# calf-ai/calfkit-sdk

Measured on NVIDIA H100. Metric: agent_events_per_sec, higher is better.
Workload: dtype u8

## Files before the change

### calfkit-sdk_b200/csrc/ck_kernels.cuh

```cuda
#ifndef CK_KERNELS_CUH
#define CK_KERNELS_CUH

#include <cuda_runtime.h>
#include "ck_walk.cuh"
#include "ck_canon.cuh"

#if !defined(__CUDA_ARCH__)
extern __shared__ uint4 ck_win_smem[];
#endif

#ifndef CK_HIST_MIN
#define CK_HIST_MIN 2048u
#endif
#ifndef CK_LONG_MIN
#define CK_LONG_MIN 16384u
#endif
struct ck_canon_ctl { unsigned long long cursor; u32 count; u32 elems; u32 cand; u32 cand_next; };
struct ck_view {
    const u8* in; const long long* off;
    const u8* ovl; const long long* ovl_off; const u32* ovl_len;
    ck_canon_ctl* canon_ctl; u32* canon_list;
    const u32* perm;
    const uint2* hist_skip;
    ck_elem* elems; u32 elem_cap;
    const u32* len;
};
__device__ __forceinline__ const u8* ck_rec_in(const ck_view& v, u32 i, u32& len) {
    long long a = v.off[i];
    len = v.len ? v.len[i] : (u32)(v.off[i + 1] - a);
    return v.in + a;
}
__device__ __forceinline__ const u8* ck_rec(const ck_view& v, u32 i, u32& len) {
    long long o = v.ovl_off[i];
    if (o >= 0) { len = v.ovl_len[i]; return v.ovl + o; }
    return ck_rec_in(v, i, len);
}

#define CK_TPL_MAX_PARTS 6
struct ck_tool_cfg {
    int32_t  publish_topic_id;
    uint32_t tpl_nparts;
    uint32_t tpl_kind[CK_TPL_MAX_PARTS];
    uint32_t tpl_off[CK_TPL_MAX_PARTS];
    uint32_t tpl_len[CK_TPL_MAX_PARTS];
    uint32_t lit_comma_q[2];
    uint32_t lit_q[2];
    uint32_t lit_open[2];
    uint32_t lit_mid[2];
    uint32_t lit_close[2];
    uint32_t lit_value_open[2];
};

struct ck_pub {
    uint32_t payload;
    int32_t  topic_id;
    uint32_t topic_off, topic_len;
    uint32_t record;
    uint32_t has_key;
    int32_t  partition;
    uint32_t pad;
};

struct ck_topic_table {
    uint32_t cap;
    const uint32_t* hash;
    const int32_t*  id;
    const uint32_t* name_off;
    const uint32_t* name_len;
    const uint8_t*  names;
};

__device__ __forceinline__ u32 ck_fnv1a(const u8* p, u32 n) {
    u32 h = 2166136261u;
    for (u32 i = 0; i < n; i++) h = (h ^ p[i]) * 16777619u;
    return h ? h : 1u;
}

#define CK_WALK_THREADS 128
template <class R>
__device__ __forceinline__ void ck_walk_one(ck_view v, u32 n, u32* __restrict__ cols, u32 stride, u32 mode) {
    u32 i = blockIdx.x * blockDim.x + threadIdx.x;
    if (i >= n) return;
    if (v.perm) i = v.perm[i];
    u32 len; const u8* rec;
    if (mode == 0) rec = ck_rec_in(v, i, len);
    else { if (v.ovl_off[i] < 0) return; rec = ck_rec(v, i, len); }
    uint2 skip = make_uint2(0u, 0u);
    if (mode == 0 && len >= CK_HIST_MIN && v.hist_skip) skip = v.hist_skip[i];
    if (skip.x == 0xffffffffu) return;
    WalkOut o; o.base = cols + i; o.stride = stride; o.skip_open = skip.x; o.skip_close = skip.y;
    u32 status, stop = 0;
    if (len == 0) status = CK_EMPTY;
    else {
        R r; r.init(rec, len);
        AnyCtx cx;
        cx.kfill = 0;
        status = ck_walk_envelope(r, o, cx, stop) ? CK_OK : (mode ? CK_UNSUPPORTED : CK_NOT_CANONICAL);
    }
    o.set(CK_COL_STATUS, status);
    o.set(CK_COL_ERR, stop);
    if (mode == 0 && status == CK_NOT_CANONICAL && v.canon_ctl) {
        u32 k = atomicAdd(&v.canon_ctl->count, 1u);
        v.canon_list[k] = i;
    }
}
#ifndef CK_WALK_MINB
#define CK_WALK_MINB 8
#endif
__global__ void __launch_bounds__(256)
ck_classify_kernel(ck_view v, u32 n, u32* __restrict__ cand) {
    u32 j = blockIdx.x * blockDim.x + threadIdx.x;
    bool take = false; u32 i = 0;
    if (j < n) { i = v.perm ? v.perm[j] : j; u32 len; ck_rec_in(v, i, len); take = len >= CK_HIST_MIN; }
    u32 m = __ballot_sync(0xffffffffu, take);
    if (!m) return;
    u32 lane = threadIdx.x & 31, base = 0;
    if (lane == (u32)(__ffs(m) - 1)) base = atomicAdd(&v.canon_ctl->cand, (u32)__popc(m));
    base = __shfl_sync(0xffffffffu, base, __ffs(m) - 1);
    if (take) cand[base + __popc(m & ((1u << lane) - 1u))] = i;
}
__global__ void __launch_bounds__(CK_WALK_THREADS, CK_WALK_MINB)
ck_walk_kernel(ck_view v, u32 n, u32* __restrict__ cols, u32 stride, u32 mode) { ck_walk_one<WRd>(v, n, cols, stride, mode); }
__global__ void __launch_bounds__(CK_WALK_THREADS, 8)
ck_walk_global_kernel(ck_view v, u32 n, u32* __restrict__ cols, u32 stride, u32 mode) { ck_walk_one<GRd>(v, n, cols, stride, mode); }

__global__ void __launch_bounds__(64)
ck_canon_kernel(ck_view v, u32 n, u32* __restrict__ cols, u32 stride, u8* __restrict__ ovl, long long ovl_cap,
                long long* __restrict__ ovl_off, u32* __restrict__ ovl_len) {
    u32 cnt = v.canon_ctl->count;
    for (u32 k = blockIdx.x * blockDim.x + threadIdx.x; k < cnt; k += gridDim.x * blockDim.x) {
        u32 i = v.canon_list[k];
        u32 len, out_len = 0;
        const u8* src = ck_rec_in(v, i, len);
        u32 st = ck_canonicalise(src, len, nullptr, 0, out_len);
        if (st != CK_OK) { cols[(size_t)CK_COL_STATUS * stride + i] = st; continue; }
        u32 need = (out_len + 15u) & ~15u;
        long long o0 = (long long)atomicAdd(&v.canon_ctl->cursor, (unsigned long long)need);
        if (o0 + need > ovl_cap) { cols[(size_t)CK_COL_STATUS * stride + i] = CK_UNSUPPORTED; continue; }
        st = ck_canonicalise(src, len, ovl + o0, need, out_len);
        if (st != CK_OK) { cols[(size_t)CK_COL_STATUS * stride + i] = CK_UNSUPPORTED; continue; }
        for (u32 b = out_len; b < need; b++) ovl[o0 + b] = 0;
        ovl_len[i] = out_len;
        ovl_off[i] = o0;
    }
}

__global__ void __launch_bounds__(64)
ck_rewalk_list_kernel(ck_view v, u32 n, u32* __restrict__ cols, u32 stride) {
    u32 cnt = v.canon_ctl->count;
    for (u32 k = blockIdx.x * blockDim.x + threadIdx.x; k < cnt; k += gridDim.x * blockDim.x) {
        u32 i = v.canon_list[k];
        if (v.ovl_off[i] < 0) continue;
        u32 len; const u8* rec = ck_rec(v, i, len);
        WalkOut o; o.base = cols + i; o.stride = stride;
        u32 stop = 0;
        GRdT r; r.init(rec, len);
        AnyCtx cx; cx.kfill = 0;
        u32 status = ck_walk_envelope(r, o, cx, stop) ? CK_OK : CK_UNSUPPORTED;
        o.set(CK_COL_STATUS, status);
        o.set(CK_COL_ERR, stop);
    }
}

__device__ __forceinline__ bool ck_span_eq(Rd& r, u32 a, u32 b, u32 len) {
    for (u32 k = 0; k < len; k++) if (r.at(a + k) != r.at(b + k)) return false;
    return true;
}

__device__ __forceinline__ Span ck_dict_find(Rd& r, u32 obj, u32 key_off, u32 key_len) {
    u32 pos = obj + 1;
    Span none = {0, 0};
    while (pos < r.n && r.at(pos) != '}') {
        Span k;
        if (!ck_string(r, pos, k)) return none;
        pos++;
        u32 v = pos;
        ck_skip_value(r, pos);
        if (k.len == key_len && ck_span_eq(r, k.off, key_off, key_len)) { Span s = {v, pos - v}; return s; }
        if (pos < r.n && r.at(pos) == ',') pos++;
    }
    return none;
}

#ifndef CK_PLAN_PF
#define CK_PLAN_PF 1
#endif
#ifndef CK_PLAN_MINB
#define CK_PLAN_MINB 1
#endif
__device__ __forceinline__ void ck_prefetch_l2(const u8* p) {
#if CK_PLAN_PF == 2
    asm volatile("prefetch.global.L1 [%0];" :: "l"(p));
#else
    asm volatile("prefetch.global.L2 [%0];" :: "l"(p));
#endif
}
#define CK_DIRECT_MIN 48u
struct SegWriter {
    ck_out_desc* d;
    Rd* r; const u8* lit; const u8* aux; u8* slot;
    u32 n, total;
    bool in_glue, overflow;
    u32 gfill, grun;
    unsigned long long acc; u32 cnt;

    __device__ __forceinline__ void init(ck_out_desc* dd, Rd* rr, const u8* l, const u8* a, u8* s) {
        d = dd; r = rr; lit = l; aux = a; slot = s; n = 0; total = 0; in_glue = false; overflow = false; gfill = 0; grun = 0; acc = 0; cnt = 0;
    }
    __device__ __forceinline__ void seg(u32 src, u32 off, u32 len) {
        if (n < CK_MAX_SEGS) { d->seg[n][0] = off; d->seg[n][1] = (len << 2) | src; n++; } else overflow = true;
    }
    __device__ __forceinline__ void put8(unsigned long long chunk, u32 nb) {
        if (gfill + nb > CK_GLUE_STRIDE) { overflow = true; return; }
        if (nb < 8) chunk &= (~0ull >> (8 * (8 - nb)));
        acc |= chunk << (8 * cnt);
        u32 c2 = cnt + nb;
        gfill += nb;
        if (c2 >= 8) {
            *(unsigned long long*)(slot + ((gfill - (c2 - 8)) - 8)) = acc;
            acc = cnt ? (chunk >> (8 * (8 - cnt))) : 0ull;
            c2 -= 8;
        }
        cnt = c2;
    }
    __device__ __forceinline__ void put(u8 b) { put8((unsigned long long)b, 1); }
    __device__ __forceinline__ static unsigned long long load8_g(const u8* p) {
        u32 s = (u32)((uintptr_t)p & 7);
        const unsigned long long* q = (const unsigned long long*)((uintptr_t)p - s);
        unsigned long long lo = q[0];
        if (s == 0) return lo;
        unsigned long long hi = q[1];
        return (lo >> (8 * s)) | (hi << (64 - 8 * s));
    }
    __device__ __forceinline__ unsigned long long fetch8(u32 src, u32 off) {
        return src == CK_SRC_INPUT ? r->load8(off) : load8_g((src == CK_SRC_LIT ? lit : aux) + off);
    }
    __device__ __forceinline__ void close_run() {
        if (cnt) { *(unsigned long long*)(slot + (gfill & ~7u)) = acc; acc = 0; cnt = 0; }
        seg(CK_SRC_GLUE, grun, gfill - grun);
        gfill = (gfill + 15u) & ~15u;
        in_glue = false;
    }
    __device__ __forceinline__ void glue_bytes(u32 src, u32 off, u32 len) {
        if (!in_glue) { in_glue = true; grun = gfill; }
        for (u32 k = 0; k < len; k += 8) put8(fetch8(src, off + k), len - k < 8 ? len - k : 8);
        total += len;
    }
    __device__ __forceinline__ void add(u32 src, u32 off, u32 len) {
        if (len == 0) return;
        bool direct_ok = (src == CK_SRC_INPUT || src == CK_SRC_AUX) && len >= CK_DIRECT_MIN;
        if (!direct_ok) { glue_bytes(src, off, len); return; }
        if (in_glue || (total & 15u)) {
            u32 need = (16u - (total & 15u)) & 15u;
            glue_bytes(src, off, need);
            off += need; len -= need;
            close_run();
        }
        u32 body = len & ~15u;
        seg(src, off, body);
        total += body;
// ... 565 lines not shown
```

### calfkit-sdk_b200/csrc/ck_walk.cuh

```cuda
#ifndef CK_WALK_CUH
#define CK_WALK_CUH

#include "ck_common.h"

#if defined(__CUDACC__)
#define CK_HD __host__ __device__ __forceinline__
#define CK_HD_NOINLINE __host__ __device__ __noinline__
#else
#define CK_HD inline __attribute__((always_inline))
#define CK_HD_NOINLINE __attribute__((noinline))
#endif

typedef uint8_t u8;
typedef uint32_t u32;
typedef uint64_t u64;
#if !defined(__CUDACC__)
struct uint4 { u32 x, y, z, w; };
#endif

struct Span { u32 off, len; };

#if defined(__CUDA_ARCH__)
extern __shared__ uint4 ck_win_smem[];
#endif
#define CK_LX_SEP 640u
#define CK_LX_CLOSE 320u
#define CK_LX_MIN 4u
#define CK_LX_KEYS 128u
#define CK_DEFER_MAX 4096u
#define CK_LX_OPEN 8u
struct ck_elem { u32 rec, start, end; };
struct ck_long_index {
    u32 n_sep[2], n_close[2], ok, rec, defer_cap, n_open;
    u32 open_sq[CK_LX_OPEN];
    ck_elem* defer_list; u32* defer_ctr;
    u32 sep[2][CK_LX_SEP];
    u32 close_[2][CK_LX_CLOSE];
    u32 kh[2][CK_LX_KEYS], koff[2][CK_LX_KEYS];
};
#if defined(__CUDA_ARCH__)
CK_HD u32 ck_lane() { return threadIdx.x & 31u; }
CK_HD bool ck_all(bool p) { return __all_sync(0xffffffffu, p); }
CK_HD u32 ck_bcast(u32 v, u32 src) { return __shfl_sync(0xffffffffu, v, src); }
CK_HD u32 ck_or_reduce(u32 v) { return __reduce_or_sync(0xffffffffu, v); }
CK_HD void ck_warp_sync() { __syncwarp(); }
CK_HD u32 ck_defer_reserve(u32* ctr, u32 n) { u32 b = 0; if ((threadIdx.x & 31u) == 0) b = atomicAdd(ctr, n); return __shfl_sync(0xffffffffu, b, 0); }
CK_HD u32 ck_max_reduce(u32 v) { return __reduce_max_sync(0xffffffffu, v); }
#else
CK_HD u32 ck_max_reduce(u32 v) { return v; }
CK_HD u32 ck_defer_reserve(u32*, u32) { return 0xffffffffu; }
CK_HD u32 ck_lane() { return 0; }
CK_HD bool ck_all(bool p) { return p; }
CK_HD u32 ck_bcast(u32 v, u32) { return v; }
CK_HD u32 ck_or_reduce(u32 v) { return v; }
CK_HD void ck_warp_sync() {}
#endif
CK_HD bool ck_lx_range(const ck_long_index* lx, u32 di, u32 pos, u32& q, u32& s0, u32& k) {
    if (!lx || !lx->ok) return false;
    u32 lo = 0, hi = lx->n_close[di];
    while (lo < hi) { u32 mid = (lo + hi) >> 1; if (lx->close_[di][mid] < pos) lo = mid + 1; else hi = mid; }
    if (lo >= lx->n_close[di]) return false;
    q = lx->close_[di][lo];
    lo = 0; hi = lx->n_sep[di];
    while (lo < hi) { u32 mid = (lo + hi) >> 1; if (lx->sep[di][mid] < pos) lo = mid + 1; else hi = mid; }
    s0 = lo;
    u32 a = lo; hi = lx->n_sep[di];
    while (a < hi) { u32 mid = (a + hi) >> 1; if (lx->sep[di][mid] < q) a = mid + 1; else hi = mid; }
    k = a - s0;
    return true;
}

struct GRd {
    static const bool kWindow = false;
    static const bool kWarp = false;
    static const bool kTrustFloats = false;
    const u8* g;
    u32 n;
    const u64* wp;
    u64 w;

    CK_HD static u64 ld64(const u64* p) {
#if defined(__CUDA_ARCH__)
        return __ldg((const unsigned long long*)p);
#else
        return *p;
#endif
    }
    CK_HD void init(const u8* base, u32 len, u32 st = 0) { (void)st; g = base; n = len; wp = nullptr; w = 0; }
    CK_HD u32 st() const { return 0; }
    CK_HD void set_st(u32) {}
    CK_HD void invalidate() {}

    CK_HD u8 at(u32 pos) {
        const u8* a = g + pos;
        const u64* q = (const u64*)((uintptr_t)a & ~(uintptr_t)7);
        if (q != wp) { wp = q; w = ld64(q); }
        return (u8)(w >> (8 * ((uintptr_t)a & 7)));
    }
    CK_HD u64 load8(u32 pos) {
        const u8* a = g + pos;
        u32 s = (u32)((uintptr_t)a & 7);
        const u64* q = (const u64*)((uintptr_t)a - s);
        u64 lo = (q == wp) ? w : ld64(q);
        if (s == 0) { wp = q; w = lo; return lo; }
        u64 hi = ld64(q + 1);
        wp = q + 1; w = hi;
        return (lo >> (8 * s)) | (hi << (64 - 8 * s));
    }
    CK_HD void load16(u32 pos, u64& x0, u64& x1) {
        const u8* a = g + pos;
        u32 s = (u32)((uintptr_t)a & 7);
        const u64* q = (const u64*)((uintptr_t)a - s);
        u64 w0 = ld64(q), w1 = ld64(q + 1);
        x0 = w0; x1 = w1;
        if (s) {
            u64 w2 = ld64(q + 2);
            x0 = (w0 >> (8 * s)) | (w1 << (64 - 8 * s));
            x1 = (w1 >> (8 * s)) | (w2 << (64 - 8 * s));
        }
    }
};

typedef GRd Rd;

struct URd : GRd {
    static const bool kWarp = true;
    u32 lock;
    CK_HD void init(const u8* base, u32 len, u32 st = 0) { GRd::init(base, len); lock = st; }
    CK_HD u32 st() const { return lock; }
    CK_HD void set_st(u32 s) { lock = s; }
    CK_HD void invalidate() {}
    CK_HD const ck_long_index* lx() const {
#if defined(__CUDA_ARCH__)
        return lock ? (const ck_long_index*)ck_win_smem + (threadIdx.x >> 5) : nullptr;
#else
        return nullptr;
#endif
    }
    CK_HD ck_long_index* lxw() const {
#if defined(__CUDA_ARCH__)
        return (ck_long_index*)ck_win_smem + (threadIdx.x >> 5);
#else
        return nullptr;
#endif
    }
};

#ifndef CK_WIN_BYTES
#define CK_WIN_BYTES 160
#endif
#define CK_WIN_BACK 16
#ifndef CK_WIN_L2PF
#define CK_WIN_L2PF 0
#endif
#define CK_WIN_STRIDE (CK_WIN_BYTES + 16)
#define CK_WIN_NONE 0x80000000u
#if defined(__CUDA_ARCH__)
extern __shared__ uint4 ck_win_smem[];
#else
static thread_local uint8_t ck_win_host[CK_WIN_STRIDE];
#endif

CK_HD_NOINLINE u32 ck_win_refill(const u8* gb, u32 ap, u32 lim) {
    u32 wb = ap & ~15u;
    wb = wb >= CK_WIN_BACK ? wb - CK_WIN_BACK : 0u;
#if defined(__CUDA_ARCH__)
    u32 dst = (u32)__cvta_generic_to_shared((const u8*)ck_win_smem + threadIdx.x * CK_WIN_STRIDE);
    const u8* src = gb + wb;
#pragma unroll
    for (u32 k = 0; k < CK_WIN_BYTES; k += 16)
        if (wb + k < lim) asm volatile("cp.async.cg.shared.global [%0], [%1], 16;" :: "r"(dst + k), "l"(src + k) : "memory");
#if CK_WIN_L2PF
    if (wb + CK_WIN_BYTES < lim) asm volatile("prefetch.global.L2 [%0];" :: "l"(src + CK_WIN_BYTES));
    if (wb + CK_WIN_BYTES + 128u < lim) asm volatile("prefetch.global.L2 [%0];" :: "l"(src + CK_WIN_BYTES + 128u));
#endif
    asm volatile("cp.async.wait_all;" ::: "memory");
#else
    for (u32 k = 0; k < CK_WIN_BYTES; k += 16) if (wb + k < lim) for (u32 j = 0; j < 16; j++) ck_win_host[k + j] = gb[wb + k + j];
#endif
    return wb;
}

struct WRd {
    static const bool kWindow = true;
    static const bool kWarp = false;
    static const bool kTrustFloats = false;
    const u8* g;
    u32 n;
    u32 wbase;
    u32 m;
    const u8* wp;

    CK_HD void init(const u8* base, u32 len, u32 st = CK_WIN_NONE) {
        g = base; n = len; wbase = st; m = (u32)((uintptr_t)base & 15);
#if defined(__CUDA_ARCH__)
        wp = (const u8*)ck_win_smem + threadIdx.x * CK_WIN_STRIDE;
#else
        wp = ck_win_host;
#endif
    }
    CK_HD u32 st() const { return wbase; }
    CK_HD void set_st(u32 s) { wbase = s; }
    CK_HD void invalidate() { wbase = CK_WIN_NONE; }
    CK_HD u32 mis() const { return m; }
    CK_HD const u8* win() const { return wp; }
    CK_HD void refill(u32 ap) { wbase = ck_win_refill(g - m, ap, (m + n + 15u) & ~15u); }
    CK_HD u8 at(u32 pos) {
        u32 ap = pos + mis();
        u32 o = ap - wbase;
        if (o >= (u32)CK_WIN_BYTES) { refill(ap); o = ap - wbase; }
        return win()[o];
    }
    CK_HD u64 load8(u32 pos) {
        u32 ap = pos + mis();
        u32 o = ap - wbase;
        if (o > (u32)(CK_WIN_BYTES - 12)) { refill(ap); o = ap - wbase; }
        const u32* w = (const u32*)(win() + (o & ~3u));
        u32 a = w[0], b = w[1], c = w[2], sh = (o & 3u) * 8u;
#if defined(__CUDA_ARCH__)
        u32 lo = __funnelshift_r(a, b, sh), hi = __funnelshift_r(b, c, sh);
#else
        u32 lo = sh ? (u32)((((u64)b << 32) | a) >> sh) : a, hi = sh ? (u32)((((u64)c << 32) | b) >> sh) : b;
#endif
        return ((u64)hi << 32) | lo;
    }
    CK_HD void load16(u32 pos, u64& x0, u64& x1) {
        u32 ap = pos + mis();
        u32 o = ap - wbase;
        if (o > (u32)(CK_WIN_BYTES - 20)) { refill(ap); o = ap - wbase; }
        const u32* w = (const u32*)(win() + (o & ~3u));
        u32 a = w[0], b = w[1], c = w[2], d = w[3], e = w[4], sh = (o & 3u) * 8u;
#if defined(__CUDA_ARCH__)
        u32 q0 = __funnelshift_r(a, b, sh), q1 = __funnelshift_r(b, c, sh), q2 = __funnelshift_r(c, d, sh), q3 = __funnelshift_r(d, e, sh);
#else
        u32 q0 = sh ? (u32)((((u64)b << 32) | a) >> sh) : a, q1 = sh ? (u32)((((u64)c << 32) | b) >> sh) : b;
        u32 q2 = sh ? (u32)((((u64)d << 32) | c) >> sh) : c, q3 = sh ? (u32)((((u64)e << 32) | d) >> sh) : d;
#endif
        x0 = ((u64)q1 << 32) | q0; x1 = ((u64)q3 << 32) | q2;
    }
};

struct WRdT : WRd { static const bool kTrustFloats = true; };
struct GRdT : GRd { static const bool kTrustFloats = true; };

#ifndef CK_PF
#define CK_PF 0
#endif
#ifndef CK_PF_DIST
#define CK_PF_DIST 256
#endif
CK_HD void ck_pf(const u8* a) {
#if defined(__CUDA_ARCH__) && CK_PF
#if CK_PF == 2
    asm volatile("prefetch.global.L1 [%0];" :: "l"(a + CK_PF_DIST));
#elif CK_PF == 4
    if (((uintptr_t)a & 127) < 32) { unsigned d; asm volatile("ld.global.ca.u32 %0, [%1];" : "=r"(d) : "l"((const void*)((uintptr_t)(a + CK_PF_DIST) & ~(uintptr_t)3))); }
#elif CK_PF == 3
    if (((uintptr_t)a & 31) < 16) asm volatile("prefetch.global.L1 [%0];" :: "l"(a + CK_PF_DIST));
#else
    if (((uintptr_t)a & 127) < 32) asm volatile("prefetch.global.L1 [%0];" :: "l"(a + CK_PF_DIST));
#endif
#else
    (void)a;
#endif
}

#define CK_REP8(b) ((u64)(b) * 0x0101010101010101ull)

CK_HD u64 ck_haszero(u64 x) { return (x - CK_REP8(0x01)) & ~x & CK_REP8(0x80); }
CK_HD u64 ck_lt20(u64 x) { return (x - CK_REP8(0x20)) & ~x & CK_REP8(0x80); }

CK_HD u32 ck_ctz64(u64 x) {
#if defined(__CUDA_ARCH__)
    return (u32)(__ffsll((long long)x) - 1);
#else
    return (u32)__builtin_ctzll(x);
#endif
}

#define CK_RET(res) (((u64)r.st() << 32) | (u64)(u32)(res))
#define CK_CALL(e, call) u64 e##64 = (call); u32 e = (u32)e##64; if (!e) { r.invalidate(); return false; } r.set_st((u32)(e##64 >> 32))

template <class R>
CK_HD_NOINLINE u32 ck_match8_core(const u8* g, u32 n, u32 pos, u32 st, u64 want, u32 nb) {
    R r; r.init(g, n, st);
    ck_pf(g + pos);
    u64 got = r.load8(pos);
    u64 mask = ~0ull >> (8 * (8 - nb));
    return (r.st() & ~1u) | (u32)(((got ^ want) & mask) == 0);
}
template <class R>
CK_HD_NOINLINE u32 ck_match16_core(const u8* g, u32 n, u32 pos, u32 st, u64 want0, u64 want1, u32 nb1) {
    R r; r.init(g, n, st);
    ck_pf(g + pos);
    u64 g0, g1;
    r.load16(pos, g0, g1);
    u64 mask1 = ~0ull >> (8 * (8 - nb1));
    return (r.st() & ~1u) | (u32)((g0 == want0) & (((g1 ^ want1) & mask1) == 0));
}
CK_HD u64 ck_lit_word(const char* lit, u32 L, u32 k) {
    u64 w = 0;
#pragma unroll
// ... 578 lines not shown
    if (!M(",\"metadata\":") || !ck_any_obj_or_null(r, pos, d + 1, cx) || !M(",\"timeout\":")) return false;
    if (PEEK('n')) { if (!ck_null(r, pos)) return false; } else if (!ck_number(r, pos, false, true)) return false;
    return M("}");
}

template <class R>
CK_HD_NOINLINE u64 ck_overrides_core(const u8* g, u32 n, u32 pos, u32 st, u32 d, AnyCtx* cxp) {
    R r; r.init(g, n, st);
    AnyCtx& cx = *cxp;
    Span t;
    if (PEEK('n')) { if (!ck_null(r, pos)) return 0; return CK_RET(pos); }
    if (!M("{\"override_agent_tools\":")) return false;
    if (PEEK('n')) { if (!ck_null(r, pos)) return false; }
    else {
        if (!M("[")) return false;
        if (!PEEK(']')) {
            for (;;) {
                if (!M("{\"node_id\":") || !ck_string(r, pos, t) || !M(",\"subscribe_topics\":[")) return false;
                if (!PEEK(']')) { for (;;) { if (!ck_string(r, pos, t)) return false; if (PEEK(',')) { pos++; continue; } break; } }
                if (!M("],\"publish_topic\":") || !ck_string_or_null(r, pos, t) || !M(",\"tool_schema\":") ||
                    !ck_tool_definition(r, pos, d + 3, cx) || !M("}")) return false;
                if (PEEK(',')) { pos++; continue; }
                break;
            }
        }
        if (!M("]")) return false;
    }
    if (!M("}")) return 0;
    return CK_RET(pos);
}
template <class R>
CK_HD bool ck_overrides_or_null(R& r, u32& pos, u32 d, AnyCtx& cx) {
    CK_CALL(e, ck_overrides_core<R>(r.g, r.n, pos, r.st(), d, &cx));
    pos = e;
    return true;
}

template <class R>
CK_HD u32 ck_content_part(R& r, u32& pos, u32 d, AnyCtx& cx, Span& val) {
    Span t;
    if (!M("{\"kind\":\"")) return 0;
    if (M("text\",\"text\":")) {
        val.off = pos;
        bool ok = ck_string(r, pos, t);
        val.len = pos - val.off;
        return (ok && M(",\"metadata\":") && ck_any_obj_or_null(r, pos, d + 1, cx) && M("}")) ? 1u : 0u;
    }
    if (M("data\",\"data\":")) {
        val.off = pos;
        bool ok = ck_any(r, pos, d + 1, cx);
        val.len = pos - val.off;
        if (!ok) return 0;
        if (!M(",\"schema_\":null,\"metadata\":")) {
            if (!R::kTrustFloats || !M(",\"schema_\":") || !ck_any(r, pos, d + 1, cx) || !M(",\"metadata\":")) return 0;
        }
        return (ck_any_obj_or_null(r, pos, d + 1, cx) && M("}")) ? 2u : 0u;
    }
    if (M("file\",\"media_type\":")) {
        return (ck_string(r, pos, t) && M(",\"uri\":") && ck_string_or_null(r, pos, t) && M(",\"data\":") &&
                ck_string_or_null(r, pos, t) && M(",\"metadata\":") && ck_any_obj_or_null(r, pos, d + 1, cx) && M("}")) ? 3u : 0u;
    }
    if (M("tool\",\"tool_call_id\":")) {
        return (ck_string(r, pos, t) && M(",\"kwargs\":") && ck_any_obj(r, pos, d + 1, cx) && M(",\"tool_name\":") &&
                ck_string(r, pos, t) && M(",\"metadata\":") && ck_any_obj_or_null(r, pos, d + 1, cx) && M("}")) ? 3u : 0u;
    }
    return 0;
}

template <class R>
CK_HD void ck_skip_value(R& r, u32& pos) {
    u32 depth = 0;
    for (;;) {
        if (pos >= r.n) return;
        u8 c = r.at(pos);
        if (c == '"') {
            pos++;
            for (;;) {
                if (pos >= r.n) return;
                u8 s = r.at(pos);
                if (s == '\\') { pos += 2; continue; }
                pos++;
                if (s == '"') break;
            }
        } else if (c == '{' || c == '[') { depth++; pos++; continue; }
        else if (c == '}' || c == ']') { depth--; pos++; }
        else if (c == ',' || c == ':') { if (depth == 0) return; pos++; continue; }
        else { pos++; while (pos < r.n) { u8 s = r.at(pos); if (s == ',' || s == '}' || s == ']' || s == ':') break; pos++; } }
        if (depth == 0) return;
    }
}

template <class R>
CK_HD_NOINLINE u64 ck_tool_result_core(const u8* g, u32 n, u32 pos, u32 st, u32 d, AnyCtx* cxp) {
    R r; r.init(g, n, st);
    AnyCtx& cx = *cxp;
    Span t;
    u32 start = pos;
    if (PEEK('{')) {
        if (M("{\"return_value\":")) {
            if (ck_any(r, pos, d + 1, cx) && M(",\"content\":") && ck_string_or_null(r, pos, t) && M(",\"metadata\":") &&
                ck_any(r, pos, d + 1, cx) && M(",\"kind\":\"tool-return\"}")) return CK_RET(pos);
        } else if (M("{\"message\":")) {
            if (ck_string(r, pos, t) && M(",\"kind\":\"model-retry\"}")) return CK_RET(pos);
        } else if (M("{\"content\":")) {
            if (ck_string(r, pos, t) && M(",\"tool_name\":") && ck_string_or_null(r, pos, t) && M(",\"tool_call_id\":") &&
                ck_string(r, pos, t) && M(",\"timestamp\":") && ck_datetime(r, pos) && M(",\"part_kind\":\"retry-prompt\"}")) {
                return CK_RET(pos);
            }
        }
        pos = start;
        if (!ck_any(r, pos, d, cx)) return false;
        u32 end = pos;
        u32 p = start + 1;
        bool have_kind = false, tagged = false, part_tagged = false;
        while (p < end && r.at(p) != '}') {
            Span k;
            if (!ck_string(r, p, k)) return false;
            p++;
            u32 v = p;
            ck_skip_value(r, p);
            bool is_kind = (k.len == 4 && r.at(k.off) == 'k' && r.at(k.off + 1) == 'i' && r.at(k.off + 2) == 'n' && r.at(k.off + 3) == 'd');
            u32 q = k.off;
            bool is_pk = (k.len == 9) && ck_match(r, q, "part_kind", 9);
            if (is_kind || is_pk) {
                u32 vv = v;
                bool tag = ck_match(r, vv, "\"tool-return\"", 13) || ck_match(r, vv, "\"model-retry\"", 13) ||
                           ck_match(r, vv, "\"retry-prompt\"", 14);
                tag = tag && (vv == p);
                if (is_kind) { have_kind = true; tagged = tag; } else part_tagged = tag;
            }
            if (p < end && r.at(p) == ',') p++;
        }
        if ((have_kind ? tagged : part_tagged) && !R::kTrustFloats) return false;
        return CK_RET(end);
    }
    if (!ck_any(r, pos, d, cx)) return 0;
    return CK_RET(pos);
}
template <class R>
CK_HD bool ck_tool_result_value(R& r, u32& pos, u32 d, AnyCtx& cx) {
    CK_CALL(e, ck_tool_result_core<R>(r.g, r.n, pos, r.st(), d, &cx));
    pos = e;
    return true;
}

struct WalkOut {
    u32* base; size_t stride; bool active = true;
    u32 skip_open = 0, skip_close = 0;
    CK_HD void set(u32 col, u32 v) { if (active) base[(size_t)col * stride] = v; }
};

#define SETSPAN(COL, a, b) do { o.set(COL, (a)); o.set(COL + 1, (b) - (a)); } while (0)

template <class R>
CK_HD bool ck_walk_envelope(R& r, WalkOut& o, AnyCtx& cx, u32& stop) {
    u32 pos = 0;
    Span t;
    stop = 0;
    u32 tc_kh_l[CK_DICT_KEYS], tc_koff_l[CK_DICT_KEYS], tc_n = 0;
    u32 tr_kh_l[CK_DICT_KEYS], tr_koff_l[CK_DICT_KEYS], tr_n = 0;
    u32 *tc_kh = tc_kh_l, *tc_koff = tc_koff_l, *tr_kh = tr_kh_l, *tr_koff = tr_koff_l;
    if constexpr (R::kWarp) {
        ck_long_index* lw = r.lxw();
        tc_kh = lw->kh[0]; tc_koff = lw->koff[0]; tr_kh = lw->kh[1]; tr_koff = lw->koff[1];
    }
    ToolCallSpans first_tc = {{0, 0}, {0, 0}, {0, 0}};
    u32 first_tc0 = 0, first_tc1 = 0, first_tr0 = 0, first_tr1 = 0;
#define FAIL do { stop = pos; return false; } while (0)
    if (!M("{\"context\":{\"state\":{\"tool_calls\":{")) FAIL;
    u32 a = pos - 1;
    if (!PEEK('}')) {
        bool par = false;
        if constexpr (R::kWarp) {
            u32 q, s0, k;
            if (ck_lx_range(r.lx(), 0, pos, q, s0, k) && k + 1 >= CK_LX_MIN) {
                par = true;
                if (k + 1 > CK_DICT_KEYS) FAIL;
                const ck_long_index* lx = r.lx();
                bool good = true;
                for (u32 base = 0; base <= k; base += 32) {
                    u32 e = base + ck_lane(), v0 = 0, v1 = 0;
                    bool ok = true;
                    ToolCallSpans tc = {{0, 0}, {0, 0}, {0, 0}};
                    if (e <= k) {
                        u32 p = e ? lx->sep[0][s0 + e - 1] + 1 : pos, tend = e == k ? q : lx->sep[0][s0 + e];
                        R lr; lr.init(r.g, r.n, 0);
                        Span key;
                        ok = ck_string(lr, p, key) && ck_match(lr, p, ":", 1);
                        v0 = p;
                        ok = ok && ck_tool_call_part(lr, p, 5, cx, tc) == 1 && p == tend;
                        v1 = p;
                        if (ok) { tc_kh[e] = ck_hash_span(lr, key.off, key.len); tc_koff[e] = key.off; }
                    }
                    good = ck_all(ok) && good;
                    if (base == 0) {
                        first_tc.tool_name.off = ck_bcast(tc.tool_name.off, 0); first_tc.tool_name.len = ck_bcast(tc.tool_name.len, 0);
                        first_tc.args.off = ck_bcast(tc.args.off, 0); first_tc.args.len = ck_bcast(tc.args.len, 0);
                        first_tc.tool_call_id.off = ck_bcast(tc.tool_call_id.off, 0); first_tc.tool_call_id.len = ck_bcast(tc.tool_call_id.len, 0);
                        first_tc0 = ck_bcast(v0, 0); first_tc1 = ck_bcast(v1, 0);
                    }
                }
                if (!good) FAIL;
                ck_warp_sync();
                bool dup = false;
                for (u32 e = ck_lane(); e <= k; e += 32) for (u32 j = 0; j < e; j++) dup |= (tc_kh[j] == tc_kh[e]);
                if (!ck_all(!dup)) FAIL;
                tc_n = k + 1; pos = q;
            }
        }
        if (!par) {
        for (;;) {
            if (!ck_string(r, pos, t)) FAIL;
            u32 h = ck_hash_span(r, t.off, t.len);
            for (u32 k = 0; k < tc_n; k++) if (tc_kh[k] == h) FAIL;
            if (tc_n >= CK_DICT_KEYS) FAIL;
            tc_kh[tc_n] = h; tc_koff[tc_n] = t.off; tc_n++;
            ToolCallSpans tc;
            if (!M(":")) FAIL;
            u32 v0 = pos;
            if (ck_tool_call_part(r, pos, 5, cx, tc) != 1) FAIL;
            if (tc_n == 1) { first_tc = tc; first_tc0 = v0; first_tc1 = pos; }
            if (PEEK(',')) { pos++; continue; }
            break;
        }
        }
    }
    if (!M("}")) FAIL;
    SETSPAN(CK_COL_TC_OFF, a, pos);

#if CK_SPEC
    bool spec_tr = M(",\"tool_results\":{},\"uncommitted_message\":null,\"message_history\":[");
    if (spec_tr) {
        u32 e = pos;
        o.set(CK_COL_TR_OFF, e - 20 - 27 - 2); o.set(CK_COL_TR_LEN, 2);
        o.set(CK_COL_UNC_OFF, e - 20 - 4); o.set(CK_COL_UNC_LEN, 4);
    } else {
#endif
    if (!M(",\"tool_results\":{")) FAIL;
    a = pos - 1;
    if (!PEEK('}')) {
        bool par = false;
        if constexpr (R::kWarp) {
            u32 q, s0, k;
            if (ck_lx_range(r.lx(), 0, pos, q, s0, k) && k + 1 >= CK_LX_MIN) {
                par = true;
                if (k + 1 > CK_DICT_KEYS) FAIL;
                const ck_long_index* lx = r.lx();
                bool good = true;
                for (u32 base = 0; base <= k; base += 32) {
                    u32 e = base + ck_lane(), v0 = 0, v1 = 0;
                    bool ok = true;
                    if (e <= k) {
                        u32 p = e ? lx->sep[0][s0 + e - 1] + 1 : pos, tend = e == k ? q : lx->sep[0][s0 + e];
                        R lr; lr.init(r.g, r.n, 0);
                        Span key;
                        ok = ck_string(lr, p, key) && ck_match(lr, p, ":", 1);
                        v0 = p;
                        ok = ok && ck_tool_result_value(lr, p, 5, cx) && p == tend;
                        v1 = p;
                        if (ok) { tr_kh[e] = ck_hash_span(lr, key.off, key.len); tr_koff[e] = key.off; }
                    }
                    good = ck_all(ok) && good;
                    if (base == 0) { first_tr0 = ck_bcast(v0, 0); first_tr1 = ck_bcast(v1, 0); }
                }
                if (!good) FAIL;
                ck_warp_sync();
                bool dup = false;
                for (u32 e = ck_lane(); e <= k; e += 32) for (u32 j = 0; j < e; j++) dup |= (tr_kh[j] == tr_kh[e]);
                if (!ck_all(!dup)) FAIL;
                tr_n = k + 1; pos = q;
            }
        }
        if (!par) {
        for (;;) {
            if (!ck_string(r, pos, t)) FAIL;
            u32 h = ck_hash_span(r, t.off, t.len);
            for (u32 k = 0; k < tr_n; k++) if (tr_kh[k] == h) FAIL;
            if (tr_n >= CK_DICT_KEYS) FAIL;
            tr_kh[tr_n] = h; tr_koff[tr_n] = t.off; tr_n++;
            if (!M(":")) FAIL;
            u32 v0 = pos;
            if (!ck_tool_result_value(r, pos, 5, cx)) FAIL;
            if (tr_n == 1) { first_tr0 = v0; first_tr1 = pos; }
            if (PEEK(',')) { pos++; continue; }
            break;
        }
        }
    }
    if (!M("}")) FAIL;
    SETSPAN(CK_COL_TR_OFF, a, pos);

    if (!M(",\"uncommitted_message\":")) FAIL;
    a = pos;
    if (PEEK('n')) { if (!ck_null(r, pos)) FAIL; } else if (!ck_message(r, pos, 4, cx)) FAIL;
    SETSPAN(CK_COL_UNC_OFF, a, pos);

    if (!M(",\"message_history\":[")) FAIL;
#if CK_SPEC
    }
#endif
    a = pos - 1;
    if (o.skip_close && o.skip_open == a) pos = o.skip_close;
    else if (!PEEK(']')) {
        bool par = false;
        if constexpr (R::kWarp) {
            u32 q, s0, k;
            if (ck_lx_range(r.lx(), 0, pos, q, s0, k)) {
                const ck_long_index* lx = r.lx();
                bool deferred = false;
                u32 longest = 0;
                for (u32 e = ck_lane(); e <= k; e += 32) { u32 a0 = e ? lx->sep[0][s0 + e - 1] + 1 : pos, a1 = e == k ? q : lx->sep[0][s0 + e]; if (a1 - a0 > longest) longest = a1 - a0; }
                if (lx->defer_list && ck_max_reduce(longest) <= CK_DEFER_MAX) {
                    u32 slot = ck_defer_reserve(lx->defer_ctr, k + 1);
                    bool fits = slot <= lx->defer_cap && k + 1 <= lx->defer_cap - slot;
                    for (u32 e = ck_lane(); e <= k; e += 32) {
                        if (slot >= lx->defer_cap || e >= lx->defer_cap - slot) break;
                        ck_elem el;
                        el.rec = fits ? lx->rec : 0xffffffffu;
                        el.start = e ? lx->sep[0][s0 + e - 1] + 1 : pos; el.end = e == k ? q : lx->sep[0][s0 + e];
                        lx->defer_list[slot + e] = el;
                    }
                    deferred = fits;
                }
                par = deferred || k + 1 >= CK_LX_MIN;
                bool good = true;
                for (u32 base = 0; par && !deferred && base <= k; base += 32) {
                    u32 e = base + ck_lane();
                    bool ok = true;
                    if (e <= k) {
                        u32 p = e ? lx->sep[0][s0 + e - 1] + 1 : pos, tend = e == k ? q : lx->sep[0][s0 + e];
                        R lr; lr.init(r.g, r.n, 0);
                        ok = ck_message(lr, p, 5, cx) != 0 && p == tend;
                    }
                    good = ck_all(ok) && good;
                }
                if (!good) FAIL;
                if (par) pos = q;
            }
        }
        if (!par) {
        for (;;) {
            if (!ck_message(r, pos, 5, cx)) FAIL;
            if (PEEK(',')) { pos++; continue; }
            break;
        }
        }
    }
    if (!M("]")) FAIL;
    SETSPAN(CK_COL_HIST_OFF, a, pos);

#if CK_SPEC
    if (M(",\"final_output_parts\":[],\"temp_instructions\":null,\"metadata\":null,\"overrides\":null},\"deps\":{\"correlation_id\":")) {
        u32 e = pos;
        o.set(CK_COL_FOP_OFF, e - 27 - 17 - 16 - 25 - 2); o.set(CK_COL_FOP_LEN, 2);
        o.set(CK_COL_ODATA_OFF, 0); o.set(CK_COL_ODATA_LEN, 0); o.set(CK_COL_OTEXT_OFF, 0); o.set(CK_COL_OTEXT_LEN, 0);
        o.set(CK_COL_TI_OFF, e - 27 - 17 - 16 - 4); o.set(CK_COL_TI_LEN, 4);
        o.set(CK_COL_SMETA_OFF, e - 27 - 17 - 4); o.set(CK_COL_SMETA_LEN, 4);
        o.set(CK_COL_SOV_OFF, e - 27 - 4); o.set(CK_COL_SOV_LEN, 4);
    } else {
#endif
    if (!M(",\"final_output_parts\":[")) FAIL;
    a = pos - 1;
    Span odata = {0, 0}, otext = {0, 0};
    if (!PEEK(']')) {
        for (;;) {
            Span val = {0, 0};
            u32 pk = ck_content_part(r, pos, 5, cx, val);
            if (!pk) FAIL;
            if (pk == 1 && otext.len == 0) otext = val;
            if (pk == 2 && odata.len == 0) odata = val;
            if (PEEK(',')) { pos++; continue; }
            break;
        }
    }
    if (!M("]")) FAIL;
    SETSPAN(CK_COL_FOP_OFF, a, pos);
    o.set(CK_COL_ODATA_OFF, odata.off); o.set(CK_COL_ODATA_LEN, odata.len);
    o.set(CK_COL_OTEXT_OFF, otext.off); o.set(CK_COL_OTEXT_LEN, otext.len);

    if (!M(",\"temp_instructions\":")) FAIL;
    a = pos;
    if (!ck_string_or_null(r, pos, t)) FAIL;
    SETSPAN(CK_COL_TI_OFF, a, pos);

    if (!M(",\"metadata\":")) FAIL;
    a = pos;
    if (!ck_any(r, pos, 4, cx)) FAIL;
    SETSPAN(CK_COL_SMETA_OFF, a, pos);

    if (!M(",\"overrides\":")) FAIL;
    a = pos;
    if (!ck_overrides_or_null(r, pos, 4, cx)) FAIL;
    SETSPAN(CK_COL_SOV_OFF, a, pos);

    if (!M("},\"deps\":{\"correlation_id\":")) FAIL;
#if CK_SPEC
    }
#endif
    if (!ck_string(r, pos, t)) FAIL;
    o.set(CK_COL_CORR_OFF, t.off); o.set(CK_COL_CORR_LEN, t.len);
    if (!M(",\"provided_deps\":")) FAIL;
    a = pos;
    if (!ck_any_obj(r, pos, 4, cx)) FAIL;
    SETSPAN(CK_COL_PD_OFF, a, pos);

    if (!M("}},\"internal_workflow_state\":{\"call_stack\":{\"_internal_list\":[")) FAIL;
    a = pos - 1;
    u32 nframes = 0;
    u32 top0 = 0, top1 = 0, fov0 = 0, fov1 = 0, top_nargs = CK_NARGS_NULL, top_kinds = 0;
    Span top_tgt = {0, 0}, top_cb = {0, 0}, top_a0 = {0, 0}, top_a1 = {0, 0};
    if (!PEEK(']')) {
        for (;;) {
            u32 f0 = pos;
            Span tgt, cb;
            if (!M("{\"target_topic\":") || !ck_string(r, pos, tgt) || !M(",\"callback_topic\":") || !ck_string(r, pos, cb)) FAIL;
            u32 nargs = CK_NARGS_NULL, kinds = 0;
            Span a0 = {0, 0}, a1 = {0, 0};
#if CK_SPEC
            if (!M(",\"input_args\":null,\"frame_id\":")) {
#endif
            if (!M(",\"input_args\":")) FAIL;
            if (PEEK('n')) { if (!ck_null(r, pos)) FAIL; }
            else {
                if (!M("[")) FAIL;
                nargs = 0;
                if (!PEEK(']')) {
                    for (;;) {
                        u32 v0 = pos;
                        Span sv;
                        bool is_str = PEEK('"');
                        if (is_str) { if (!ck_string(r, pos, sv)) FAIL; }
                        else { if (!ck_any(r, pos, 6, cx)) FAIL; sv.off = v0; sv.len = pos - v0; }
                        if (nargs == 0) { a0 = sv; kinds |= is_str ? 1u : 0u; }
                        if (nargs == 1) { a1 = sv; kinds |= is_str ? 2u : 0u; }
                        nargs++;
                        if (PEEK(',')) { pos++; continue; }
                        break;
                    }
                }
                if (!M("]")) FAIL;
            }
            if (!M(",\"frame_id\":")) FAIL;
#if CK_SPEC
            }
#endif
            if (!ck_string(r, pos, t)) FAIL;
            u32 ov0, ov1;
#if CK_SPEC
            if (M(",\"overrides\":null}")) { ov1 = pos - 1; ov0 = ov1 - 4; } else
#endif
            {
                if (!M(",\"overrides\":")) FAIL;
                ov0 = pos;
                if (!ck_overrides_or_null(r, pos, 6, cx)) FAIL;
                ov1 = pos;
                if (!M("}")) FAIL;
            }
            nframes++;
            top0 = f0; top1 = pos; fov0 = ov0; fov1 = ov1; top_nargs = nargs; top_kinds = kinds;
            top_tgt = tgt; top_cb = cb; top_a0 = a0; top_a1 = a1;
            if (PEEK(',')) { pos++; continue; }
            break;
        }
    }
    SETSPAN(CK_COL_TOP_OFF, top0, top1);
    o.set(CK_COL_TGT_OFF, top_tgt.off); o.set(CK_COL_TGT_LEN, top_tgt.len);
    o.set(CK_COL_CB_OFF, top_cb.off); o.set(CK_COL_CB_LEN, top_cb.len);
    o.set(CK_COL_NARGS, top_nargs); o.set(CK_COL_ARGKINDS, top_kinds);
    o.set(CK_COL_ARG0_OFF, top_a0.off); o.set(CK_COL_ARG0_LEN, top_a0.len);
    o.set(CK_COL_ARG1_OFF, top_a1.off); o.set(CK_COL_ARG1_LEN, top_a1.len);
    SETSPAN(CK_COL_FOV_OFF, fov0, fov1);
#if CK_SPEC
    if (M("]},\"metadata\":null}}")) {
        u32 e = pos;
        o.set(CK_COL_FRAMES_OFF, a); o.set(CK_COL_FRAMES_LEN, e - 19 - a);
        o.set(CK_COL_NFRAMES, nframes);
        o.set(CK_COL_WFMETA_OFF, e - 6); o.set(CK_COL_WFMETA_LEN, 4);
    } else {
#endif
    if (!M("]")) FAIL;
    SETSPAN(CK_COL_FRAMES_OFF, a, pos);
    o.set(CK_COL_NFRAMES, nframes);
    if (!M("},\"metadata\":")) FAIL;
    a = pos;
    if (!ck_any(r, pos, 3, cx)) FAIL;
    SETSPAN(CK_COL_WFMETA_OFF, a, pos);
    if (!M("}}")) FAIL;
#if CK_SPEC
    }
#endif
    if (pos != r.n) FAIL;
    u32 call0 = 0, call1 = 0, res0 = 0, res1 = 0;
    Span tn = {0, 0}, ar = {0, 0};
    if (nframes > 0 && top_nargs == 2 && (top_kinds & 1u)) {
        u32 h = ck_hash_span(r, top_a0.off, top_a0.len);
        GRd gr, gq; gr.init(r.g, r.n); gq.init(r.g, r.n);
        for (u32 k = 0; k < tc_n; k++) {
            if (tc_kh[k] != h) continue;
            u32 ko = tc_koff[k];
            if (ko + top_a0.len >= r.n || gr.at(ko + top_a0.len) != '"') continue;
            if (!ck_spans_equal(gr, ko, gq, top_a0.off, top_a0.len)) continue;
            if (k == 0) { call0 = first_tc0; call1 = first_tc1; tn = first_tc.tool_name; ar = first_tc.args; break; }
            u32 p2 = ko + top_a0.len + 2;
            call0 = p2;
            ToolCallSpans tcs;
            ck_tool_call_part(r, p2, 5, cx, tcs);
            call1 = p2; tn = tcs.tool_name; ar = tcs.args;
            break;
        }
        for (u32 k = 0; k < tr_n; k++) {
            if (tr_kh[k] != h) continue;
            u32 ko = tr_koff[k];
            if (ko + top_a0.len >= r.n || gr.at(ko + top_a0.len) != '"') continue;
            if (!ck_spans_equal(gr, ko, gq, top_a0.off, top_a0.len)) continue;
            if (k == 0) { res0 = first_tr0; res1 = first_tr1; break; }
            u32 p2 = ko + top_a0.len + 2;
            res0 = p2;
            ck_tool_result_value(r, p2, 5, cx);
            res1 = p2;
            break;
        }
    }
    SETSPAN(CK_COL_CALL_VAL_OFF, call0, call1);
    o.set(CK_COL_TNAME_OFF, tn.off); o.set(CK_COL_TNAME_LEN, tn.len);
    o.set(CK_COL_ARGS_OFF, ar.off); o.set(CK_COL_ARGS_LEN, ar.len);
    SETSPAN(CK_COL_RES_OFF, res0, res1);
    return true;
#undef FAIL
}

#endif
```

Before: 310.3 million.

## Keep first dict keys in registers, rescan overflow keys; widen smem window

Replaces the per-thread local-memory arrays of tool-call and tool-result key hashes with a small register-resident dictionary holding the first two keys. Any keys beyond that are found by re-parsing the JSON from a saved offset instead of being stored. The warp path still uses shared memory. It also enlarges the per-thread shared read window and lowers the walk kernel's min-blocks-per-SM bound, trading occupancy for more registers and fewer refills. The intent is to cut local-memory spills and traffic, at the cost of re-scanning the input for records with many keys.

Measured after the change: 336.9 million (median of 6 runs). 1.09x the previous value.

```diff
diff --git a/calfkit-sdk_b200/csrc/ck_kernels.cuh b/calfkit-sdk_b200/csrc/ck_kernels.cuh
--- a/calfkit-sdk_b200/csrc/ck_kernels.cuh
+++ b/calfkit-sdk_b200/csrc/ck_kernels.cuh
@@ -105,7 +105,7 @@
     }
 }
 #ifndef CK_WALK_MINB
-#define CK_WALK_MINB 8
+#define CK_WALK_MINB 6
 #endif
 __global__ void __launch_bounds__(256)
 ck_classify_kernel(ck_view v, u32 n, u32* __restrict__ cand) {
diff --git a/calfkit-sdk_b200/csrc/ck_walk.cuh b/calfkit-sdk_b200/csrc/ck_walk.cuh
--- a/calfkit-sdk_b200/csrc/ck_walk.cuh
+++ b/calfkit-sdk_b200/csrc/ck_walk.cuh
@@ -147,7 +147,7 @@
 };
 
 #ifndef CK_WIN_BYTES
-#define CK_WIN_BYTES 160
+#define CK_WIN_BYTES 224
 #endif
 #define CK_WIN_BACK 16
 #ifndef CK_WIN_L2PF
@@ -1032,18 +1032,83 @@
 
 #define SETSPAN(COL, a, b) do { o.set(COL, (a)); o.set(COL + 1, (b) - (a)); } while (0)
 
+CK_HD bool ck_key_is(const u8* g, u32 n, u32 ko, u32 a, u32 len) {
+    GRd gr, gq; gr.init(g, n); gq.init(g, n);
+    if (ko + len >= n || gr.at(ko + len) != '"') return false;
+    return ck_spans_equal(gr, ko, gq, a, len);
+}
+
+#ifndef CK_DICT_REG
+#define CK_DICT_REG 2
+#endif
+template <class R, bool kShared = R::kWarp>
+struct DictKeys {
+    u32 kh[CK_DICT_REG], koff[CK_DICT_REG];
+    u32 n;
+    u32 more;
+    CK_HD void init(u32*, u32*) { n = 0; more = 0; }
+    template <class F>
+    CK_HD bool scan_more(R& r, u32 h, F fn) {
+        u32 p = more;
+        for (u32 k = CK_DICT_REG; k < n; k++) {
+            u32 q = p;
+            ck_skip_value(r, p);
+            if (ck_hash_span(r, q + 1, p - q - 2) == h && fn(q + 1)) return true;
+            p++;
+            ck_skip_value(r, p);
+            p++;
+        }
+        return false;
+    }
+    CK_HD bool add(R& r, u32 h, u32 off) {
+        bool dup = false;
+#pragma unroll
+        for (u32 k = 0; k < CK_DICT_REG; k++) dup |= (k < n) & (kh[k] == h);
+        if (dup || n >= CK_DICT_KEYS) return false;
+        if (n > CK_DICT_REG && scan_more(r, h, [](u32) { return true; })) return false;
+#pragma unroll
+        for (u32 k = 0; k < CK_DICT_REG; k++) if (k == n) { kh[k] = h; koff[k] = off; }
+        if (n == CK_DICT_REG) more = off - 1;
+        n++;
+        return true;
+    }
+    CK_HD u32 find(R& r, u32 h, u32 a, u32 len, u32& ko) {
+#pragma unroll
+        for (u32 k = 0; k < CK_DICT_REG; k++)
+            if (k < n && kh[k] == h && ck_key_is(r.g, r.n, koff[k], a, len)) { ko = koff[k]; return k; }
+        u32 hit = ~0u;
+        if (n > CK_DICT_REG) scan_more(r, h, [&](u32 off) { if (!ck_key_is(r.g, r.n, off, a, len)) return false; ko = off; hit = CK_DICT_REG; return true; });
+        return hit;
+    }
+};
+template <class R>
+struct DictKeys<R, true> {
+    u32 *kh, *koff;
+    u32 n;
+    CK_HD void init(u32* h, u32* off) { kh = h; koff = off; n = 0; }
+    CK_HD bool add(R&, u32 h, u32 off) {
+        for (u32 k = 0; k < n; k++) if (kh[k] == h) return false;
+        if (n >= CK_DICT_KEYS) return false;
+        kh[n] = h; koff[n] = off; n++;
+        return true;
+    }
+    CK_HD u32 find(R& r, u32 h, u32 a, u32 len, u32& ko) {
+        for (u32 k = 0; k < n; k++)
+            if (kh[k] == h && ck_key_is(r.g, r.n, koff[k], a, len)) { ko = koff[k]; return k; }
+        return ~0u;
+    }
+};
+
 template <class R>
 CK_HD bool ck_walk_envelope(R& r, WalkOut& o, AnyCtx& cx, u32& stop) {
     u32 pos = 0;
     Span t;
     stop = 0;
-    u32 tc_kh_l[CK_DICT_KEYS], tc_koff_l[CK_DICT_KEYS], tc_n = 0;
-    u32 tr_kh_l[CK_DICT_KEYS], tr_koff_l[CK_DICT_KEYS], tr_n = 0;
-    u32 *tc_kh = tc_kh_l, *tc_koff = tc_koff_l, *tr_kh = tr_kh_l, *tr_koff = tr_koff_l;
+    DictKeys<R> tck, trk;
     if constexpr (R::kWarp) {
         ck_long_index* lw = r.lxw();
-        tc_kh = lw->kh[0]; tc_koff = lw->koff[0]; tr_kh = lw->kh[1]; tr_koff = lw->koff[1];
-    }
+        tck.init(lw->kh[0], lw->koff[0]); trk.init(lw->kh[1], lw->koff[1]);
+    } else { tck.init(nullptr, nullptr); trk.init(nullptr, nullptr); }
     ToolCallSpans first_tc = {{0, 0}, {0, 0}, {0, 0}};
     u32 first_tc0 = 0, first_tc1 = 0, first_tr0 = 0, first_tr1 = 0;
 #define FAIL do { stop = pos; return false; } while (0)
@@ -1070,7 +1135,7 @@
                         v0 = p;
                         ok = ok && ck_tool_call_part(lr, p, 5, cx, tc) == 1 && p == tend;
                         v1 = p;
-                        if (ok) { tc_kh[e] = ck_hash_span(lr, key.off, key.len); tc_koff[e] = key.off; }
+                        if (ok) { tck.kh[e] = ck_hash_span(lr, key.off, key.len); tck.koff[e] = key.off; }
                     }
                     good = ck_all(ok) && good;
                     if (base == 0) {
@@ -1083,23 +1148,20 @@
                 if (!good) FAIL;
                 ck_warp_sync();
                 bool dup = false;
-                for (u32 e = ck_lane(); e <= k; e += 32) for (u32 j = 0; j < e; j++) dup |= (tc_kh[j] == tc_kh[e]);
+                for (u32 e = ck_lane(); e <= k; e += 32) for (u32 j = 0; j < e; j++) dup |= (tck.kh[j] == tck.kh[e]);
                 if (!ck_all(!dup)) FAIL;
-                tc_n = k + 1; pos = q;
+                tck.n = k + 1; pos = q;
             }
         }
         if (!par) {
         for (;;) {
             if (!ck_string(r, pos, t)) FAIL;
-            u32 h = ck_hash_span(r, t.off, t.len);
-            for (u32 k = 0; k < tc_n; k++) if (tc_kh[k] == h) FAIL;
-            if (tc_n >= CK_DICT_KEYS) FAIL;
-            tc_kh[tc_n] = h; tc_koff[tc_n] = t.off; tc_n++;
+            if (!tck.add(r, ck_hash_span(r, t.off, t.len), t.off)) FAIL;
             ToolCallSpans tc;
             if (!M(":")) FAIL;
             u32 v0 = pos;
             if (ck_tool_call_part(r, pos, 5, cx, tc) != 1) FAIL;
-            if (tc_n == 1) { first_tc = tc; first_tc0 = v0; first_tc1 = pos; }
+            if (tck.n == 1) { first_tc = tc; first_tc0 = v0; first_tc1 = pos; }
             if (PEEK(',')) { pos++; continue; }
             break;
         }
@@ -1138,7 +1200,7 @@
                         v0 = p;
                         ok = ok && ck_tool_result_value(lr, p, 5, cx) && p == tend;
                         v1 = p;
-                        if (ok) { tr_kh[e] = ck_hash_span(lr, key.off, key.len); tr_koff[e] = key.off; }
+                        if (ok) { trk.kh[e] = ck_hash_span(lr, key.off, key.len); trk.koff[e] = key.off; }
                     }
                     good = ck_all(ok) && good;
                     if (base == 0) { first_tr0 = ck_bcast(v0, 0); first_tr1 = ck_bcast(v1, 0); }
@@ -1146,22 +1208,19 @@
                 if (!good) FAIL;
                 ck_warp_sync();
                 bool dup = false;
-                for (u32 e = ck_lane(); e <= k; e += 32) for (u32 j = 0; j < e; j++) dup |= (tr_kh[j] == tr_kh[e]);
+                for (u32 e = ck_lane(); e <= k; e += 32) for (u32 j = 0; j < e; j++) dup |= (trk.kh[j] == trk.kh[e]);
                 if (!ck_all(!dup)) FAIL;
-                tr_n = k + 1; pos = q;
+                trk.n = k + 1; pos = q;
             }
         }
         if (!par) {
         for (;;) {
             if (!ck_string(r, pos, t)) FAIL;
-            u32 h = ck_hash_span(r, t.off, t.len);
-            for (u32 k = 0; k < tr_n; k++) if (tr_kh[k] == h) FAIL;
-            if (tr_n >= CK_DICT_KEYS) FAIL;
-            tr_kh[tr_n] = h; tr_koff[tr_n] = t.off; tr_n++;
+            if (!trk.add(r, ck_hash_span(r, t.off, t.len), t.off)) FAIL;
             if (!M(":")) FAIL;
             u32 v0 = pos;
             if (!ck_tool_result_value(r, pos, 5, cx)) FAIL;
-            if (tr_n == 1) { first_tr0 = v0; first_tr1 = pos; }
+            if (trk.n == 1) { first_tr0 = v0; first_tr1 = pos; }
             if (PEEK(',')) { pos++; continue; }
             break;
         }
@@ -1374,31 +1433,23 @@
     Span tn = {0, 0}, ar = {0, 0};
     if (nframes > 0 && top_nargs == 2 && (top_kinds & 1u)) {
         u32 h = ck_hash_span(r, top_a0.off, top_a0.len);
-        GRd gr, gq; gr.init(r.g, r.n); gq.init(r.g, r.n);
-        for (u32 k = 0; k < tc_n; k++) {
-            if (tc_kh[k] != h) continue;
-            u32 ko = tc_koff[k];
-            if (ko + top_a0.len >= r.n || gr.at(ko + top_a0.len) != '"') continue;
-            if (!ck_spans_equal(gr, ko, gq, top_a0.off, top_a0.len)) continue;
-            if (k == 0) { call0 = first_tc0; call1 = first_tc1; tn = first_tc.tool_name; ar = first_tc.args; break; }
+        u32 ko = 0;
+        u32 k = tck.find(r, h, top_a0.off, top_a0.len, ko);
+        if (k == 0) { call0 = first_tc0; call1 = first_tc1; tn = first_tc.tool_name; ar = first_tc.args; }
+        else if (k != ~0u) {
             u32 p2 = ko + top_a0.len + 2;
             call0 = p2;
             ToolCallSpans tcs;
             ck_tool_call_part(r, p2, 5, cx, tcs);
             call1 = p2; tn = tcs.tool_name; ar = tcs.args;
-            break;
-        }
-        for (u32 k = 0; k < tr_n; k++) {
-            if (tr_kh[k] != h) continue;
-            u32 ko = tr_koff[k];
-            if (ko + top_a0.len >= r.n || gr.at(ko + top_a0.len) != '"') continue;
-            if (!ck_spans_equal(gr, ko, gq, top_a0.off, top_a0.len)) continue;
-            if (k == 0) { res0 = first_tr0; res1 = first_tr1; break; }
+        }
+        k = trk.find(r, h, top_a0.off, top_a0.len, ko);
+        if (k == 0) { res0 = first_tr0; res1 = first_tr1; }
+        else if (k != ~0u) {
             u32 p2 = ko + top_a0.len + 2;
             res0 = p2;
             ck_tool_result_value(r, p2, 5, cx);
             res1 = p2;
-            break;
         }
     }
     SETSPAN(CK_COL_CALL_VAL_OFF, call0, call1);
```
